# ziyangwang007/CV-SSL-MIS

Hardware: AMD Instinct MI355X
Metric: training images-or-volumes/sec/node (Mean-Teacher step) (higher is better)
Workload: dtype f32

## Files before the change

### cv-ssl-mis_amd/csrc/conv_wino.hip

```cpp
#include "common.h"
#include "wino.h"
#include <stdio.h>
#include <stdlib.h>
#include <type_traits>

namespace {

using namespace mis_dma;
using namespace mis_wino;

struct WinoArgs {
    const float* x; long long x_bs;
    const float* wt;
    const float* bias;
    float* y; long long y_bs;
    int N, Cin, Cout, D, H, W;
    int nci4;
    int boxes_z, boxes_y, boxes_x, co_groups;
    unsigned n_blocks, n_blocks_padded;
    float2* stat; long long stat_sc, stat_sn;
    const float* xn; long long xn_bs;
    const float* thr;
    float slope;
    int ks; long long y_ks;
};

template <int GZ_, int GY_, int GX_, int WZ_, int WY_, int WX_, int COB_, int NBUF_, int DW_ = 0, int FLAT_ = 0>
struct WinoCfg {
    static constexpr int GZ = GZ_, GY = GY_, GX = GX_, WZ = WZ_, WY = WY_, WX = WX_, COB = COB_, NBUF = NBUF_, FLAT = FLAT_;
    static constexpr int BZ = GZ * WZ, BY = GY * WY, BX = GX * WX;
    static constexpr int OZ = 2 * BZ, OY = 2 * BY, OX = 2 * BX;
    static constexpr int HZ = OZ + 2, HY = OY + 2;
    static constexpr int DW = DW_;
    static constexpr int NQ = DW ? OX + 2 : (OX + 8) / 4, RX = DW ? OX + 2 : NQ * 4, X0 = DW ? 0 : 3;
    static constexpr int GROUPS = HZ * HY * NQ;
    static constexpr int NCH = (GROUPS + 63) / 64;
    static constexpr int CS_RAW = DW ? NCH * 64 : GROUPS * 4;
    static constexpr int CS = CS_RAW + (49 - CS_RAW % 64 + 64) % 64;
    static constexpr int IN_FLOATS = 4 * CS;
    static constexpr int W_FLOATS = COB * 4096;
    static constexpr int STAGE = IN_FLOATS + W_FLOATS;
    static constexpr int MAX_COUT = 384;
    static constexpr int LDS_BYTES = NBUF * STAGE * 4 + 512 + MAX_COUT * 4 + NCH * 256;
    static constexpr int WPW = COB * 4;
    static constexpr int P = NCH + WPW;
    static_assert(FLAT ? (GZ * GY * GX <= 64 && WZ * WY * WX == 1 && COB == 1 && DW == 1) : (GZ * GY * GX == 16), "16 tiles per wave");
    static_assert(FLAT || WZ * WY * WX * COB == 4, "4 waves");
    static_assert(NBUF == 3 || NBUF == 4, "ring depth");
    static_assert(2 * P <= 63 && P <= 21, "vmcnt range (two stages in flight), DMA slots");
    static_assert(LDS_BYTES <= 160 * 1024, "LDS");
};

#ifndef MIS_WINO_DBG_CT
#define MIS_WINO_DBG_CT 0
#endif
#ifndef MIS_WINO_NV
#define MIS_WINO_NV 16
#endif
constexpr int NVP = MIS_WINO_NV;
constexpr int DBG = MIS_WINO_DBG_CT;

extern __shared__ __attribute__((aligned(16))) float mis_wino_lds[];

template <class C>
struct Issue {
    unsigned voff[C::NCH];
    unsigned wvoff[C::WPW];
    i32x4 rx, rw;
    unsigned st;
    unsigned cbase;
    unsigned wbase;

    template <int I>
    __device__ __forceinline__ void piece(int wave) const {
        if constexpr (I >= 0 && I < C::NCH && !(DBG & 256)) {
            if constexpr (C::DW) {
                dma_dword_s(st + (unsigned)(wave * C::CS + I * 64) * 4u, voff[I], cbase, rx);
            } else if (I * 64 + 64 <= C::GROUPS || I * 64 + (int)(threadIdx.x & 63) < C::GROUPS) {
                dma_dwordx4_s(st + (unsigned)(wave * C::CS + I * 256) * 4u, voff[I], cbase, rx);
            }
        } else if constexpr (I >= C::NCH && I < C::P && !(DBG & 128)) {
            dma_dwordx4_s(st + (unsigned)(C::IN_FLOATS + (wave + 4 * (I - C::NCH)) * 256) * 4u, wvoff[I - C::NCH], wbase, rw);
        }
    }
    template <int I, int END>
    __device__ __forceinline__ void pieces(int wave) const {
        if constexpr (I < END) { piece<I>(wave); pieces<I + 1, END>(wave); }
    }
};

typedef const __attribute__((address_space(3))) float* lds_ptr;
struct RawPlanes { lds_ptr z[4]; };

template <class C, bool FIRST, int K>
__device__ __forceinline__ void slots(const f32x4* __restrict__ wl, const f32x4* __restrict__ wl_next,
                                      const RawPlanes& raw, const f32x2 (&cur)[32], f32x2 (&nxt)[32],
                                      f32x4 (&acc)[64], f32x4 (&ar)[4], const Issue<C>& is, int wave) {
    if constexpr (K < 64) {
        constexpr int G = K / 4;
        if constexpr (K % 4 == 0 && !(DBG & 32)) ar[(G + 2) % 4] = G < 14 ? wl[(G + 2) * 64] : wl_next[(G - 14) * 64];
        {
            const float av = ar[G % 4][K % 4], bv = cur[K / 2][K % 2];
            if constexpr (K < NVP) {
                if constexpr (FIRST) asm volatile("v_mfma_f32_16x16x4_f32 %0, %1, %2, 0" : "=v"(acc[K]) : "v"(av), "v"(bv));
                else asm volatile("v_mfma_f32_16x16x4_f32 %0, %1, %2, %0" : "+v"(acc[K]) : "v"(av), "v"(bv));
            } else {
                if constexpr (FIRST) asm volatile("v_mfma_f32_16x16x4_f32 %0, %1, %2, 0" : "=a"(acc[K]) : "v"(av), "v"(bv));
                else asm volatile("v_mfma_f32_16x16x4_f32 %0, %1, %2, %0" : "+a"(acc[K]) : "v"(av), "v"(bv));
            }
        }
        if constexpr (K < 16 && !(DBG & 16)) {
#pragma unroll
            for (int j = 2 * K; j < 2 * K + 2; ++j) {
                const int z = j / 8, y = (j / 2) % 4, xp = j % 2;
                nxt[j] = f32x2{raw.z[z][y * C::RX + 2 * xp], raw.z[z][y * C::RX + 2 * xp + 1]};
            }
        }
        constexpr int SP = C::P <= 12 ? 5 : 3;
        if constexpr (K >= 2 && (K - 2) % SP == 0 && (K - 2) / SP < C::P && !(DBG & 8)) is.template piece<(K - 2) / SP>(wave);
        if constexpr (K >= 16 && K < 40 && !(DBG & 16) && (DBG & 512)) in_unit<K - 16>(nxt);
        __builtin_amdgcn_sched_barrier(0);
        slots<C, FIRST, K + 1>(wl, wl_next, raw, cur, nxt, acc, ar, is, wave);
    }
}

template <class C, bool NB, bool SPLIT>
__device__ __forceinline__ void wino_fwd_body(const WinoArgs& a) {
    float* const lds = mis_wino_lds;
    const int xcd = blockIdx.x % MIS_NUM_XCD, slot = blockIdx.x / MIS_NUM_XCD, nslot = gridDim.x / MIS_NUM_XCD;
    const unsigned per = a.n_blocks_padded / MIS_NUM_XCD;
    const unsigned box_end = (xcd + 1) * per < a.n_blocks ? (xcd + 1) * per : a.n_blocks;
    unsigned box = xcd * per + slot;
    if (box >= box_end) return;

    const int tid = threadIdx.x, lane = tid & 63;
    const int wave = __builtin_amdgcn_readfirstlane(tid >> 6);
    const int lk = lane >> 4, lj = lane & 15;
    const int cb = wave % C::COB, grp = wave / C::COB;
    int tx, ty, tz;
    bool lane_live = true;
    if constexpr (C::FLAT) {
        int t = grp * 16 + lj;
        lane_live = t < C::BZ * C::BY * C::BX;
        t = lane_live ? t : 0;
        tx = t % C::BX; ty = (t / C::BX) % C::BY; tz = t / (C::BX * C::BY);
    } else {
        const int gx = grp % C::WX, gy = (grp / C::WX) % C::WY, gz = grp / (C::WX * C::WY);
        tx = gx * C::GX + lj % C::GX; ty = gy * C::GY + (lj / C::GX) % C::GY; tz = gz * C::GZ + lj / (C::GX * C::GY);
    }
    const long long S = (long long)a.D * a.H * a.W;
    const unsigned s_bytes = (unsigned)S * 4u;
    const unsigned lds0 = lds_addr(lds);
    const int nst = SPLIT ? a.nci4 / a.ks : a.nci4;

    struct Box { int cg, kz, bx, by, bz, n, z0, y0, x0; long long idx; };
    auto finish = [&](Box& b) {
        b.z0 = b.bz * C::OZ; b.y0 = b.by * C::OY; b.x0 = b.bx * C::OX;
        b.idx = ((long long)b.bz * a.boxes_y + b.by) * a.boxes_x + b.bx;
    };
    auto decode = [&](unsigned L) {
        Box b;
        unsigned t = L;
        b.cg = t % a.co_groups; t /= a.co_groups;
        b.kz = 0;
        if constexpr (SPLIT) { b.kz = t % a.ks; t /= a.ks; }
        b.bx = t % a.boxes_x;   t /= a.boxes_x;
        b.by = t % a.boxes_y;   t /= a.boxes_y;
        b.bz = t % a.boxes_z;   t /= a.boxes_z;
        b.n = t;
        finish(b);
        return b;
    };
    const Box stride = decode((unsigned)nslot);
    auto advance = [&](Box b) {
        int c;
        b.cg += stride.cg;     c = b.cg >= a.co_groups; b.cg -= c ? a.co_groups : 0;
        if constexpr (SPLIT) { b.kz += stride.kz + c; c = b.kz >= a.ks; b.kz -= c ? a.ks : 0; }
        b.bx += stride.bx + c; c = b.bx >= a.boxes_x;   b.bx -= c ? a.boxes_x : 0;
        b.by += stride.by + c; c = b.by >= a.boxes_y;   b.by -= c ? a.boxes_y : 0;
        b.bz += stride.bz + c; c = b.bz >= a.boxes_z;   b.bz -= c ? a.boxes_z : 0;
        b.n += stride.n + c;
        finish(b);
        return b;
    };

    Issue<C> is;
    is.rw = make_rsrc(a.wt, (unsigned)a.co_groups * C::COB * (unsigned)a.nci4 * 16384u);
#pragma unroll
    for (int i = 0; i < C::WPW; ++i) {
        const int j = wave + 4 * i, b = j / 16, pp = j % 16;
        is.wvoff[i] = (unsigned)((b * a.nci4) * 4096 + pp * 256 + lane * 4) * 4u;
    }
    int icg = 0, ikz = 0;
    unsigned* const s_geo = reinterpret_cast<unsigned*>(lds + C::NBUF * C::STAGE + 128 + C::MAX_COUT);
    if (tid < 64) {
#pragma unroll
        for (int p = 0; p < C::NCH; ++p) {
            const int e = p * 64 + tid;
            const int row = e / C::NQ, q = e - row * C::NQ;
            const int hz = row / C::HY, hy = row - hz * C::HY;
            s_geo[p * 64 + tid] = (unsigned)(hz | hy << 4 | q << 9 | (e < C::GROUPS ? 1 << 14 : 0));
        }
    }
    __syncthreads();
    auto cursor_box = [&](const Box& b_in, bool live) {
        Box b = b_in;
        if (DBG & 2048) { b.n = 0; b.z0 = 0; b.y0 = 0; b.x0 = 0; }
        icg = b.cg; ikz = b.kz;
        is.rx = make_rsrc(a.x + (long long)b.n * a.x_bs, live ? (unsigned)a.Cin * s_bytes : 0u);
        unsigned geo[C::NCH];
#pragma unroll
        for (int p = 0; p < C::NCH; ++p) geo[p] = s_geo[p * 64 + lane];
        __builtin_amdgcn_sched_barrier(0);
#pragma unroll
        for (int p = 0; p < C::NCH; ++p) {
            const unsigned g = geo[p];
            const int qz = b.z0 - 1 + (int)(g & 15u), qy = b.y0 - 1 + (int)((g >> 4) & 31u);
            const int qx = C::DW ? b.x0 - 1 + (int)((g >> 9) & 31u) : b.x0 - 4 + 4 * (int)((g >> 9) & 31u);
            const bool ok = (g >> 14) && (unsigned)qz < (unsigned)a.D && (unsigned)qy < (unsigned)a.H &&
                            (unsigned)qx < (unsigned)a.W;
            is.voff[p] = ok ? (unsigned)((qz * a.H + qy) * a.W + qx) * 4u : OOB;
        }
    };
    auto cursor_set = [&](unsigned gs_issue, int istage) {
        is.st = lds0 + (gs_issue % C::NBUF) * (unsigned)(C::STAGE * 4);
        if constexpr (SPLIT) istage += ikz * nst;
        is.cbase = (unsigned)(istage * 4 + wave) * s_bytes;
        is.wbase = (unsigned)(icg * C::COB * a.nci4 + istage) * 16384u;
    };

    const int poff = ((2 * tz) * C::HY + 2 * ty) * C::RX + C::X0 + 2 * tx + lk * C::CS;
    auto raw_of = [&](unsigned gs) { return lds + (gs % C::NBUF) * C::STAGE + poff; };
    auto wl_of = [&](unsigned gs) {
        return reinterpret_cast<const f32x4*>(lds + (gs % C::NBUF) * C::STAGE + C::IN_FLOATS + cb * 4096) + lane;
    };

    float* const s_bias = lds + C::NBUF * C::STAGE + 128;
    if constexpr (NB) {
        for (int i = tid; i < a.N * a.Cout; i += 256) s_bias[i] = a.thr[i];
    } else {
        for (int i = tid; i < a.Cout; i += 256) s_bias[i] = a.bias ? a.bias[i] : 0.f;
    }
    constexpr int A = C::NBUF - 1;
    const unsigned nslot_u = (unsigned)nslot;
    Box bb = decode(box), nb = bb;
    cursor_box(bb, true);
#pragma unroll
    for (int s = 0; s < A; ++s) { cursor_set((unsigned)s, s); is.template pieces<0, C::P>(wave); }
    static_assert(A == 3, "the waits below are written for a ring of 4");
    vmwait<2 * C::P>::go();
    __syncthreads();
    f32x2 ua[32], ub[32];
    f32x4 acc[64];
    f32x4 ar[4];
    {
        const float* __restrict__ raw = raw_of(0);
#pragma unroll
        for (int j = 0; j < 32; ++j) {
            const int z = j / 8, y = (j / 2) % 4, xp = j % 2;
            ua[j] = f32x2{raw[(z * C::HY + y) * C::RX + 2 * xp], raw[(z * C::HY + y) * C::RX + 2 * xp + 1]};
        }
    }
    ar[0] = wl_of(0)[0]; ar[1] = wl_of(0)[64];
    in_units<0, 24>(ua);
    vmwait<C::P>::go();
    __syncthreads();

    unsigned gs = 0;
    const int sw = nst - A;
    auto iter = [&](auto first, f32x2 (&cur)[32], f32x2 (&nxt)[32], int s, bool relaxed) {
        cursor_set(gs + A, s + A < nst ? s + A : s + A - nst);
        RawPlanes rp;
        {
            const float* r0 = raw_of(gs + 1);
#pragma unroll
            for (int z = 0; z < 4; ++z) {
                rp.z[z] = (lds_ptr)r0 + z * C::HY * C::RX;
                asm volatile("" : "+v"(rp.z[z]));
            }
        }
        slots<C, decltype(first)::value, 0>(wl_of(gs), wl_of(gs + 1), rp, cur, nxt, acc, ar, is, wave);
        if (!(DBG & 16) && !(DBG & 512)) in_units<0, 24>(nxt);
        ++gs;
        if (NB && relaxed) vmwait<C::P + 16>::go();
        else vmwait<(DBG & 1024) ? 2 * C::P : C::P>::go();
        if (!(DBG & 64)) __syncthreads();
    };

    float run1[4] = {0.f, 0.f, 0.f, 0.f}, run2[4] = {0.f, 0.f, 0.f, 0.f};
    f32x2 xv[NB ? 16 : 1];
    for (; box < box_end; box += nslot_u, bb = nb) {
        const bool nlive = box + nslot_u < box_end;
        nb = advance(bb);
        if (sw == 0 && !(DBG & 4)) cursor_box(nb, nlive);
        iter(std::true_type{}, ua, ub, 0, false);
        if (sw == 1 && !(DBG & 4)) cursor_box(nb, nlive);
        iter(std::false_type{}, ub, ua, 1, false);
        for (int s = 2; s < nst; s += 2) {
            if (sw == s && !(DBG & 4)) cursor_box(nb, nlive);
            if constexpr (NB) {
                if (s + 2 >= nst && !(DBG & 4096)) {
                    const int oz = bb.z0 + 2 * tz, oy = bb.y0 + 2 * ty, ox = bb.x0 + 2 * tx;
                    const bool okx = lane_live && oz < a.D && oy < a.H && ox < a.W;
                    const int c0 = (bb.cg * C::COB + cb) * 16;
                    const i32x4 rxn = make_rsrc(a.xn + (long long)bb.n * a.xn_bs + (long long)c0 * S, 16u * s_bytes);
                    const unsigned vx = okx ? (unsigned)(lk * 4) * s_bytes + (unsigned)((oz * a.H + oy) * a.W + ox) * 4u : OOB;
                    unsigned vzy[4];
#pragma unroll
                    for (int zy = 0; zy < 4; ++zy) vzy[zy] = vx + (unsigned)(((zy >> 1) * a.H + (zy & 1)) * a.W) * 4u;
#pragma unroll
                    for (int r = 0; r < 4; ++r) {
                        const unsigned so = (unsigned)r * s_bytes;
#pragma unroll
                        for (int zy = 0; zy < 4; ++zy)
                            asm volatile("buffer_load_dwordx2 %0, %1, %2, %3 offen"
                                         : "=v"(xv[r * 4 + zy]) : "v"(vzy[zy]), "s"(rxn), "s"(so) : "memory");
                    }
                }
            }
            iter(std::false_type{}, ua, ub, s, NB && s + 2 >= nst);
            if (sw == s + 1 && !(DBG & 4)) cursor_box(nb, nlive);
            iter(std::false_type{}, ub, ua, s + 1, false);
        }

        if constexpr (NB) {
#pragma unroll
            for (int i = 0; i < 16; ++i) asm volatile("" : "+v"(xv[i]));
        }
        if (DBG & 2) continue;
        asm volatile("s_nop 15\n\ts_nop 15" ::: "memory");
        const int oz = bb.z0 + 2 * tz, oy = bb.y0 + 2 * ty, ox = bb.x0 + 2 * tx;
        const bool ok = lane_live && oz < a.D && oy < a.H && ox < a.W;
        const int co0 = (bb.cg * C::COB + cb) * 16;
        const __amdgpu_buffer_rsrc_t ry = __builtin_amdgcn_make_buffer_rsrc(
            (void*)(a.y + (SPLIT ? (long long)bb.kz * a.y_ks : 0LL) + (long long)bb.n * a.y_bs + (long long)co0 * S), 0,
            (int)(16u * s_bytes), 0x00020000);
        const unsigned vo = ok && !(DBG & 1) ? (unsigned)(lk * 4) * s_bytes + (unsigned)((oz * a.H + oy) * a.W + ox) * 4u : OOB;
#pragma unroll
        for (int h = 0; h < 2; ++h) {
            f32x2 o[2][2][2];
#pragma unroll
            for (int x = 0; x < 4; ++x) {
                f32x2 py[2][2];
#pragma unroll
                for (int y = 0; y < 4; ++y) {
                    const f32x2 m0 = (y * 4 + x < NVP) ? f32x2{acc[y * 4 + x][2 * h], acc[y * 4 + x][2 * h + 1]} : acc_pair(acc[y * 4 + x], h),
                                m1 = acc_pair(acc[16 + y * 4 + x], h),
                                m2 = acc_pair(acc[32 + y * 4 + x], h), m3 = acc_pair(acc[48 + y * 4 + x], h);
                    const f32x2 pz0 = m0 + m1 + m2, pz1 = m1 - m2 - m3;
                    if (y == 0) { py[0][0] = pz0; py[1][0] = pz1; }
                    if (y == 1) { py[0][0] += pz0; py[1][0] += pz1; py[0][1] = pz0; py[1][1] = pz1; }
                    if (y == 2) { py[0][0] += pz0; py[1][0] += pz1; py[0][1] -= pz0; py[1][1] -= pz1; }
                    if (y == 3) { py[0][1] -= pz0; py[1][1] -= pz1; }
                    __builtin_amdgcn_sched_barrier(0);
                }
#pragma unroll
                for (int zz = 0; zz < 2; ++zz)
#pragma unroll
                    for (int yy = 0; yy < 2; ++yy) {
                        if (x == 0) { o[zz][yy][0] = py[zz][yy]; }
                        if (x == 1) { o[zz][yy][0] += py[zz][yy]; o[zz][yy][1] = py[zz][yy]; }
                        if (x == 2) { o[zz][yy][0] += py[zz][yy]; o[zz][yy][1] -= py[zz][yy]; }
                        if (x == 3) { o[zz][yy][1] -= py[zz][yy]; }
                    }
                __builtin_amdgcn_sched_barrier(0);
            }
            f32x2 bv = *reinterpret_cast<const f32x2*>(s_bias + (NB ? bb.n * a.Cout : 0) + co0 + lk * 4 + 2 * h);
            const f32x2 th = bv;
            if constexpr (NB) bv = f32x2{0.f, 0.f};
            f32x2 s1 = {0.f, 0.f}, s2 = s1;
#pragma unroll
            for (int zz = 0; zz < 2; ++zz)
#pragma unroll
                for (int yy = 0; yy < 2; ++yy) {
                    const f32x2 v0 = o[zz][yy][0] + bv, v1 = o[zz][yy][1] + bv;
                    if constexpr (NB && !(DBG & 8192)) {
#pragma unroll
                        for (int rr = 0; rr < 2; ++rr) {
                            const f32x2 x = xv[(2 * h + rr) * 4 + zz * 2 + yy];
                            const float d0 = x[0] > th[rr] ? v0[rr] : v0[rr] * a.slope;
                            const float d1 = x[1] > th[rr] ? v1[rr] : v1[rr] * a.slope;
                            s1[rr] += d0 + d1;
                            s2[rr] = fmaf(d0, x[0], fmaf(d1, x[1], s2[rr]));
                        }
                    } else {
                        s1 += v0 + v1;
                        s2 += v0 * v0 + v1 * v1;
                    }
#pragma unroll
                    for (int rr = 0; rr < 2; ++rr) {
                        typedef unsigned u32x2 __attribute__((ext_vector_type(2)));
                        const f32x2 v = {v0[rr], v1[rr]};
                        __builtin_amdgcn_raw_buffer_store_b64(__builtin_bit_cast(u32x2, v), ry,
                                                              (int)(vo + (unsigned)((zz * a.H + yy) * a.W) * 4u),
                                                              (int)((unsigned)(2 * h + rr) * s_bytes), 0);
                    }
                }
            if constexpr (C::DW) {
                if (!ok) { s1 = f32x2{0.f, 0.f}; s2 = s1; }
            }
            run1[2 * h] += s1[0]; run1[2 * h + 1] += s1[1]; run2[2 * h] += s2[0]; run2[2 * h + 1] += s2[1];
            __builtin_amdgcn_sched_barrier(0);
        }
        const bool flush = !nlive || nb.n != bb.n || nb.cg != bb.cg;
        if (a.stat && !flush) {
            if (tid < C::COB * 16)
                a.stat[(long long)(bb.cg * C::COB * 16 + tid) * a.stat_sc + (long long)bb.n * a.stat_sn + bb.idx] = make_float2(0.f, 0.f);
        } else if (a.stat) {
            float st1[4], st2[4];
#pragma unroll
            for (int r = 0; r < 4; ++r) { st1[r] = run1[r]; st2[r] = run2[r]; run1[r] = 0.f; run2[r] = 0.f; }
#pragma unroll
            for (int r = 0; r < 4; ++r)
#pragma unroll
                for (int o = 1; o < 16; o <<= 1) {
                    st1[r] += __shfl_xor(st1[r], o, 64);
                    st2[r] += __shfl_xor(st2[r], o, 64);
                }
            float2* red = reinterpret_cast<float2*>(lds + C::NBUF * C::STAGE);
            if (lj == 0) {
#pragma unroll
                for (int r = 0; r < 4; ++r) red[wave * 16 + lk * 4 + r] = make_float2(st1[r], st2[r]);
            }
            __syncthreads();
            if (tid < C::COB * 16) {
                const int b = tid / 16, c = tid % 16;
                float sx = 0.f, sq = 0.f;
#pragma unroll
                for (int g = 0; g < 4 / C::COB; ++g) {
                    const float2 p = red[(g * C::COB + b) * 16 + c];
                    sx += p.x; sq += p.y;
                }
                a.stat[(long long)((bb.cg * C::COB + b) * 16 + c) * a.stat_sc + (long long)bb.n * a.stat_sn + bb.idx] =
                    make_float2(sx, sq);
            }
        }
    }
}

template <class C, bool NB = false>
__global__ __launch_bounds__(256) __attribute__((amdgpu_waves_per_eu(1, 1))) void wino_fwd_kernel(const WinoArgs a) {
    wino_fwd_body<C, NB, false>(a);
}
template <class C>
__global__ __launch_bounds__(256) __attribute__((amdgpu_waves_per_eu(1, 1))) void wino_fwd_split_kernel(const WinoArgs a) {
    wino_fwd_body<C, false, true>(a);
}

template <class C, bool NB = false, bool SPLIT = false>
int launch_wino(WinoArgs a, hipStream_t stream) {
    a.boxes_z = (int)mis_cdiv(a.D, C::OZ);
    a.boxes_y = (int)mis_cdiv(a.H, C::OY);
    a.boxes_x = (int)mis_cdiv(a.W, C::OX);
    a.co_groups = a.Cout / (16 * C::COB);
    const long long nb = (long long)a.N * a.boxes_z * a.boxes_y * a.boxes_x * a.co_groups * (SPLIT ? a.ks : 1);
    if (nb <= 0 || nb > 0x7fffffffLL) return MIS_ERR_ARG;
    a.n_blocks = (unsigned)nb;
    a.n_blocks_padded = (unsigned)(mis_cdiv(nb, MIS_NUM_XCD) * MIS_NUM_XCD);
    static std::atomic<unsigned long long> attr_done{0};
    const unsigned grid = a.n_blocks_padded < 256u ? a.n_blocks_padded : 256u;
    if constexpr (SPLIT) {
        if (mis_set_lds_attr(reinterpret_cast<const void*>(&wino_fwd_split_kernel<C>), C::LDS_BYTES, attr_done) != MIS_OK)
            return MIS_ERR_LAUNCH;
        hipLaunchKernelGGL((wino_fwd_split_kernel<C>), dim3(grid), dim3(256), C::LDS_BYTES, stream, a);
    } else {
        if (mis_set_lds_attr(reinterpret_cast<const void*>(&wino_fwd_kernel<C, NB>), C::LDS_BYTES, attr_done) != MIS_OK)
            return MIS_ERR_LAUNCH;
        hipLaunchKernelGGL((wino_fwd_kernel<C, NB>), dim3(grid), dim3(256), C::LDS_BYTES, stream, a);
    }
    return mis_launch_status();
}

using WinoV2 = WinoCfg<1, 4, 4, 4, 1, 1, 1, 4, 1>;
using WinoV3 = WinoCfg<3, 3, 6, 1, 1, 1, 1, 4, 1, 1>;

int wino_splits(int N, int Cin, int Cout, int D, int H, int W, int variant) {
    static const bool on = [] { const char* e = getenv("MIS_WINO_SPLIT"); return !(e && e[0] == '0'); }();
    if (!on || (variant != 2 && variant != 3)) return 1;
    const long long boxes = variant == 2 ? mis_cdiv(D, 8) * mis_cdiv(H, 8) * mis_cdiv(W, 8) : (long long)(D / 6) * (H / 6) * (W / 12);
    const long long entries = (long long)N * boxes * (Cout / 16);
    const int nst = (Cin + 3) / 4;
    int ks = 1;
    while (entries * ks < 192 && ks < 8 && nst % (2 * ks) == 0 && nst / (2 * ks) >= 8 && (nst / (2 * ks)) % 2 == 0) ks *= 2;
    return ks;
}

__global__ __launch_bounds__(256) void wino_split_reduce_kernel(const float* __restrict__ part, long long part_ks, long long part_bs,
                                                                const float* __restrict__ bias, float* __restrict__ y,
                                                                long long y_bs, int Cout, int S, int ks, float2* stat,
                                                                long long stat_sc, long long stat_sn, int tiles) {
    __shared__ float2 red[256];
    const int n = blockIdx.x / Cout, c = blockIdx.x - n * Cout;
    const float* __restrict__ p = part + (long long)n * part_bs + (long long)c * S;
    float* __restrict__ o = y + (long long)n * y_bs + (long long)c * S;
    const float b = bias ? bias[c] : 0.f;
    float s1 = 0.f, s2 = 0.f;
    for (int v = threadIdx.x; v < S; v += 256) {
        float acc = p[v];
        for (int k = 1; k < ks; ++k) acc += p[(long long)k * part_ks + v];
        acc += b;
        o[v] = acc;
        s1 += acc; s2 = fmaf(acc, acc, s2);
    }
    if (!stat) return;
    red[threadIdx.x] = make_float2(s1, s2);
    __syncthreads();
    for (int w = 128; w > 0; w >>= 1) {
        if ((int)threadIdx.x < w) { red[threadIdx.x].x += red[threadIdx.x + w].x; red[threadIdx.x].y += red[threadIdx.x + w].y; }
        __syncthreads();
    }
    for (int t = threadIdx.x; t < tiles; t += 256)
        stat[(long long)c * stat_sc + (long long)n * stat_sn + t] = t == 0 ? red[0] : make_float2(0.f, 0.f);
}

}

extern "C" int mis_conv3d_wino_select(int N, int Cin, int Cout, int D, int H, int W) {
    if (N <= 0 || Cin < 16 || Cin % 8 || Cout <= 0 || Cout % 16 || Cout > 384 || D <= 0 || H <= 0 || W <= 0) return -1;
    if (D % 2 || H % 2 || W % 2) return -1;
    if (((long long)Cin + 32) * D * H * W * 4 >= (1LL << 30)) return -1;
    if (W % 32 == 0 && D % 4 == 0 && H % 4 == 0) return 0;
    if (W % 16 == 0 && D % 4 == 0 && H % 8 == 0) return 1;
    if (W % 8 == 0 && D % 8 == 0 && H % 8 == 0 && Cin >= 32) return 2;
    if (W == 12 && D % 6 == 0 && H % 6 == 0 && Cin >= 32 &&
        (long long)N * (D / 6) * (H / 6) * (Cout / 16) * wino_splits(N, Cin, Cout, D, H, W, 3) >= 64) return 3;
    if (Cin >= 32) {
        const long long boxes = mis_cdiv(D, 8) * mis_cdiv(H, 8) * mis_cdiv(W, 8);
        if ((long long)D * H * W * 5 >= boxes * 512 * 2 && (long long)N * boxes * (Cout / 16) * wino_splits(N, Cin, Cout, D, H, W, 2) >= 128)
            return 2;
    }
    return -1;
}

namespace {
template <class C>
long long boxes_per_image(int D, int H, int W) {
    return mis_cdiv(D, C::OZ) * mis_cdiv(H, C::OY) * mis_cdiv(W, C::OX);
}
}

extern "C" long long mis_conv3d_wino_stat_tiles(int D, int H, int W, int variant) {
    if (D <= 0 || H <= 0 || W <= 0) return MIS_ERR_ARG;
    if (variant == 0) return boxes_per_image<WinoCfg<1, 1, 16, 2, 2, 1, 1, 4>>(D, H, W);
    if (variant == 1) return boxes_per_image<WinoCfg<1, 2, 8, 2, 2, 1, 1, 4>>(D, H, W);
    if (variant == 2) return boxes_per_image<WinoCfg<1, 4, 4, 4, 1, 1, 1, 4, 1>>(D, H, W);
    if (variant == 3) return boxes_per_image<WinoCfg<3, 3, 6, 1, 1, 1, 1, 4, 1, 1>>(D, H, W);
    return MIS_ERR_UNSUPPORTED;
}

extern "C" int mis_conv3d_wino_kernel_name(int variant, char* name, int name_len) {
    if (!name || name_len <= 0) return MIS_ERR_ARG;
    if (variant == 0) snprintf(name, name_len, "wino_fwd_kernel<WinoCfg<1, 1, 16, 2, 2, 1, 1, 4, 0, 0>, false>");
    else if (variant == 1) snprintf(name, name_len, "wino_fwd_kernel<WinoCfg<1, 2, 8, 2, 2, 1, 1, 4, 0, 0>, false>");
    else if (variant == 2) snprintf(name, name_len, "wino_fwd_kernel<WinoCfg<1, 4, 4, 4, 1, 1, 1, 4, 1, 0>, false>");
    else if (variant == 3) snprintf(name, name_len, "wino_fwd_kernel<WinoCfg<3, 3, 6, 1, 1, 1, 1, 4, 1, 1>, false>");
    else return MIS_ERR_UNSUPPORTED;
    return MIS_OK;
}

extern "C" int mis_conv3d_wino_fwd(const float* x, long long x_bs, const float* wt, const float* bias, float* y,
                                   long long y_bs, int N, int Cin, int Cout, int D, int H, int W, float* stat,
                                   long long stat_sc, long long stat_sn, int variant, hipStream_t stream) {
    if (!x || !wt || !y || N <= 0 || Cin <= 0 || Cout <= 0 || D <= 0 || H <= 0 || W <= 0) return MIS_ERR_ARG;
    const long long S = (long long)D * H * W;
    if (x_bs < (long long)Cin * S || y_bs < (long long)Cout * S) return MIS_ERR_ARG;
    if (Cout % 16 || Cout > 384 || Cin % 8 || Cin < 16 || (W % 4 && variant < 2) || D % 2 || H % 2 || W % 2 || y_bs % 2 || ((uintptr_t)y & 7) || ((uintptr_t)wt & 15))
        return MIS_ERR_UNSUPPORTED;
    if (((long long)Cin + 32) * S * 4 >= (1LL << 30)) return MIS_ERR_UNSUPPORTED;
    WinoArgs a{};
    a.x = x; a.x_bs = x_bs; a.wt = wt; a.bias = bias; a.y = y; a.y_bs = y_bs;
    a.N = N; a.Cin = Cin; a.Cout = Cout; a.D = D; a.H = H; a.W = W;
    a.nci4 = (Cin + 3) / 4;
    a.stat = reinterpret_cast<float2*>(stat); a.stat_sc = stat_sc; a.stat_sn = stat_sn;
    if (variant == 0) return launch_wino<WinoCfg<1, 1, 16, 2, 2, 1, 1, 4>>(a, stream);
    if (variant == 1) return launch_wino<WinoCfg<1, 2, 8, 2, 2, 1, 1, 4>>(a, stream);
    if (variant == 2) return launch_wino<WinoCfg<1, 4, 4, 4, 1, 1, 1, 4, 1>>(a, stream);
    if (variant == 3) {
        if (W != 12 || D % 6 || H % 6) return MIS_ERR_UNSUPPORTED;
        return launch_wino<WinoCfg<3, 3, 6, 1, 1, 1, 1, 4, 1, 1>>(a, stream);
    }
    return MIS_ERR_UNSUPPORTED;
}

extern "C" int mis_conv3d_wino_fwd_splits(int N, int Cin, int Cout, int D, int H, int W, int variant) {
    if (N <= 0 || Cin <= 0 || Cout <= 0 || D <= 0 || H <= 0 || W <= 0 || variant < 0 || variant > 3) return MIS_ERR_ARG;
    return wino_splits(N, Cin, Cout, D, H, W, variant);
}
extern "C" long long mis_conv3d_wino_fwd_workspace_bytes(int N, int Cin, int Cout, int D, int H, int W, int variant) {
    const int ks = mis_conv3d_wino_fwd_splits(N, Cin, Cout, D, H, W, variant);
    if (ks < 0) return ks;
    return ks > 1 ? (long long)ks * N * Cout * D * H * W * 4 : 0;
}

extern "C" int mis_conv3d_wino_fwd_ws(const float* x, long long x_bs, const float* wt, const float* bias, float* y,
                                      long long y_bs, int N, int Cin, int Cout, int D, int H, int W, float* stat,
                                      long long stat_sc, long long stat_sn, int variant, float* workspace,
                                      long long workspace_bytes, hipStream_t stream) {
    const int ks = mis_conv3d_wino_fwd_splits(N, Cin, Cout, D, H, W, variant);
    if (ks < 0) return ks;
    if (ks == 1)
        return mis_conv3d_wino_fwd(x, x_bs, wt, bias, y, y_bs, N, Cin, Cout, D, H, W, stat, stat_sc, stat_sn, variant, stream);
    if (!x || !wt || !y || !workspace) return MIS_ERR_ARG;
    const long long S = (long long)D * H * W;
    if (x_bs < (long long)Cin * S || y_bs < (long long)Cout * S) return MIS_ERR_ARG;
    if (Cout % 16 || Cout > 384 || Cin % 8 || Cin < 16 || D % 2 || H % 2 || W % 2 || ((uintptr_t)workspace & 15) || ((uintptr_t)wt & 15))
        return MIS_ERR_UNSUPPORTED;
    if (variant == 3 && (W != 12 || D % 6 || H % 6)) return MIS_ERR_UNSUPPORTED;
    if (((long long)Cin + 32) * S * 4 >= (1LL << 30)) return MIS_ERR_UNSUPPORTED;
    if (workspace_bytes < (long long)ks * N * Cout * S * 4) return MIS_ERR_WORKSPACE;
    WinoArgs a{};
    a.x = x; a.x_bs = x_bs; a.wt = wt; a.bias = nullptr; a.y = workspace; a.y_bs = (long long)Cout * S;
    a.N = N; a.Cin = Cin; a.Cout = Cout; a.D = D; a.H = H; a.W = W;
    a.nci4 = (Cin + 3) / 4;
    a.ks = ks; a.y_ks = (long long)N * Cout * S;
    const int st = variant == 2 ? launch_wino<WinoV2, false, true>(a, stream) : launch_wino<WinoV3, false, true>(a, stream);
    if (st) return st;
    const int tiles = (int)mis_conv3d_wino_stat_tiles(D, H, W, variant);
    hipLaunchKernelGGL(wino_split_reduce_kernel, dim3((unsigned)(N * Cout)), dim3(256), 0, stream, workspace, a.y_ks, a.y_bs, bias, y,
                       y_bs, Cout, (int)S, ks, reinterpret_cast<float2*>(stat), stat_sc, stat_sn, tiles);
    return mis_launch_status();
}

extern "C" int mis_conv3d_wino_dgrad_norm(const float* dy, long long dy_bs, const float* wt, float* da, long long da_bs,
                                          int N, int Cin, int Cout, int D, int H, int W, const float* xn, long long xn_bs,
                                          const float* mean, float slope, float* part, long long part_sc,
                                          long long part_sn, int variant, hipStream_t stream) {
    if (!dy || !wt || !da || !xn || !mean || !part || N <= 0 || Cin <= 0 || Cout <= 0 || D <= 0 || H <= 0 || W <= 0)
        return MIS_ERR_ARG;
    const long long S = (long long)D * H * W;
    if (dy_bs < (long long)Cin * S || da_bs < (long long)Cout * S || xn_bs < (long long)Cout * S) return MIS_ERR_ARG;
    if (variant < 0 || variant > 1 || (long long)N * Cout > 384) return MIS_ERR_UNSUPPORTED;
    if (Cout % 16 || Cin % 8 || Cin < 16 || W % 4 || D % 2 || H % 2 || da_bs % 2 || xn_bs % 2 || ((uintptr_t)da & 7) ||
        ((uintptr_t)xn & 7) || ((uintptr_t)wt & 15))
        return MIS_ERR_UNSUPPORTED;
    if (mis_conv3d_wino_select(N, Cin, Cout, D, H, W) != variant) return MIS_ERR_UNSUPPORTED;
    if (((long long)Cin + 32) * S * 4 >= (1LL << 30) || 16 * S * 4 >= (1LL << 31)) return MIS_ERR_UNSUPPORTED;
    WinoArgs a{};
    a.x = dy; a.x_bs = dy_bs; a.wt = wt; a.bias = nullptr; a.y = da; a.y_bs = da_bs;
    a.N = N; a.Cin = Cin; a.Cout = Cout; a.D = D; a.H = H; a.W = W;
    a.nci4 = (Cin + 3) / 4;
    a.stat = reinterpret_cast<float2*>(part); a.stat_sc = part_sc; a.stat_sn = part_sn;
    a.xn = xn; a.xn_bs = xn_bs; a.thr = mean; a.slope = slope;
    if (variant == 0) return launch_wino<WinoCfg<1, 1, 16, 2, 2, 1, 1, 4>, true>(a, stream);
    return launch_wino<WinoCfg<1, 2, 8, 2, 2, 1, 1, 4>, true>(a, stream);
}
```

### include/mis_hip.h

```cpp
#ifndef MIS_HIP_H
#define MIS_HIP_H

#include <stdint.h>

#ifdef __cplusplus
extern "C" {
#endif

#define MIS_OK 0
#define MIS_ERR_ARG (-1)
#define MIS_ERR_UNSUPPORTED (-2)
#define MIS_ERR_LAUNCH (-3)
#define MIS_ERR_WORKSPACE (-4)

#ifdef MIS_HIP_BUILD
typedef hipStream_t mis_stream_t;
#else
typedef void* mis_stream_t;
#endif

typedef struct MisStepState {
    uint64_t seed;
    uint64_t offset;
    int64_t iter_num;
    float lr;
    float ema_alpha;
    float cons_weight;
    float cons_gate;
} MisStepState;

int mis_abi_version(void);

int mis_conv_cin_pad(int cin);
int mis_conv_cout_pad(int cout);
long long mis_conv_packed_floats(int Cout, int Cin, int taps, int mode);
int mis_conv_pack_weights(const float* w, float* wp, int Cout, int Cin, int taps, int mode, mis_stream_t stream);
int mis_conv_pack_job_bytes(void);
long long mis_conv_pack_job(void* job_out, const float* w, float* wp, int Cout, int Cin, int taps, int mode,
                            long long start);
int mis_conv_pack_batch(const void* jobs_device, int n, long long total_floats, mis_stream_t stream);
int mis_conv_fwd(const float* x, long long x_bs, const float* wp, const float* bias, float* y, long long y_bs,
                 int N, int Cin, int Cout, int D, int H, int W, int kd, int kh, int kw, mis_stream_t stream);
long long mis_conv_fwd_stat_tiles(int N, int Cin, int Cout, int D, int H, int W, int kd, int kh, int kw);
int mis_conv_fwd_stats(const float* x, long long x_bs, const float* wp, const float* bias, float* y, long long y_bs,
                       int N, int Cin, int Cout, int D, int H, int W, int kd, int kh, int kw, float* stat,
                       long long stat_sc, long long stat_sn, mis_stream_t stream);
int mis_norm_stats_finalize(const float* part, int N, int C, long long S, int tiles, int per_sample, float eps,
                            float* mean, float* rstd, float* running_mean, float* running_var,
                            long long* num_batches_tracked, float momentum, mis_stream_t stream);
int mis_conv_fwd_kernel_name(int N, int Cin, int Cout, int D, int H, int W, int kd, int kh, int kw, char* name,
                             int name_len);
int mis_conv3d_wino_select(int N, int Cin, int Cout, int D, int H, int W);
long long mis_conv3d_wino_stat_tiles(int D, int H, int W, int variant);
int mis_conv3d_wino_kernel_name(int variant, char* name, int name_len);
int mis_conv3d_wino_fwd(const float* x, long long x_bs, const float* wt, const float* bias, float* y, long long y_bs,
                        int N, int Cin, int Cout, int D, int H, int W, float* stat, long long stat_sc,
                        long long stat_sn, int variant, mis_stream_t stream);
int mis_conv3d_wino_fwd_splits(int N, int Cin, int Cout, int D, int H, int W, int variant);
long long mis_conv3d_wino_fwd_workspace_bytes(int N, int Cin, int Cout, int D, int H, int W, int variant);
int mis_conv3d_wino_fwd_ws(const float* x, long long x_bs, const float* wt, const float* bias, float* y, long long y_bs,
                           int N, int Cin, int Cout, int D, int H, int W, float* stat, long long stat_sc, long long stat_sn,
                           int variant, float* workspace, long long workspace_bytes, mis_stream_t stream);
int mis_conv3d_wino_dgrad_norm(const float* dy, long long dy_bs, const float* wt, float* da, long long da_bs, int N,
                               int Cin, int Cout, int D, int H, int W, const float* xn, long long xn_bs,
                               const float* mean, float slope, float* part, long long part_sc, long long part_sn,
                               int variant, mis_stream_t stream);
int mis_conv2d_wino_select(int N, int Cin, int Cout, int H, int W);
long long mis_conv2d_wino_stat_tiles(int H, int W, int variant);
int mis_conv2d_wino_kernel_name(int variant, char* name, int name_len);
int mis_conv2d_wino_fwd(const float* x, long long x_bs, const float* wt, const float* bias, float* y, long long y_bs,
                        int N, int Cin, int Cout, int H, int W, float* stat, long long stat_sc, long long stat_sn,
                        int variant, mis_stream_t stream);
int mis_conv2d_wino_wgrad_select(int N, int Cin, int Cout, int H, int W);
int mis_conv2d_wino_wgrad_kernel_name(int variant, char* name, int name_len);
long long mis_conv2d_wino_wgrad_workspace_bytes(int N, int Cin, int Cout, int H, int W, int variant);
int mis_conv2d_wino_wgrad(const float* x, long long x_bs, const float* dy, long long dy_bs, float* dw, float* workspace,
                          long long workspace_bytes, int N, int Cin, int Cout, int H, int W, int accumulate, int variant,
                          mis_stream_t stream);
int mis_conv3d_wino_wgrad_select(int N, int Cin, int Cout, int D, int H, int W);
int mis_conv3d_wino_wgrad_kernel_name(int variant, char* name, int name_len);
long long mis_conv3d_wino_wgrad_workspace_bytes(int N, int Cin, int Cout, int D, int H, int W, int variant);
int mis_conv3d_wino_wgrad(const float* x, long long x_bs, const float* dy, long long dy_bs, float* dw, float* workspace,
                          long long workspace_bytes, int N, int Cin, int Cout, int D, int H, int W, int accumulate,
                          int variant, mis_stream_t stream);
long long mis_conv_wgrad_workspace_bytes(int N, int Cin, int Cout, int D, int H, int W, int kd, int kh, int kw);
int mis_conv_wgrad_kernel_name(int N, int Cin, int Cout, int D, int H, int W, int kd, int kh, int kw, char* name,
                               int name_len);
int mis_conv_wgrad(const float* x, long long x_bs, const float* dy, long long dy_bs, float* dw, float* workspace,
                   long long workspace_bytes, int N, int Cin, int Cout, int D, int H, int W, int kd, int kh,
                   int kw, int accumulate, mis_stream_t stream);
int mis_channel_sum(const float* x, long long x_bs, int N, int C, long long S, float* out, int accumulate,
                    void* workspace, long long workspace_bytes, mis_stream_t stream);

long long mis_norm_workspace_bytes(int N, int C, long long S, int per_sample);
int mis_norm_stats(const float* x, long long x_bs, int N, int C, long long S, int per_sample, float eps,
                   float* mean, float* rstd, float* running_mean, float* running_var,
                   long long* num_batches_tracked, float momentum, void* workspace, long long workspace_bytes,
                   mis_stream_t stream);
int mis_norm_stats_from_running(const float* running_mean, const float* running_var, float eps, float* mean,
                                float* rstd, int C, mis_stream_t stream);
int mis_norm_act_fwd(const float* x, long long x_bs, float* y, long long y_bs, int N, int C, long long S,
                     int per_sample, const float* mean, const float* rstd, const float* gamma, const float* beta,
                     float slope, float drop_p, unsigned drop_salt, const MisStepState* state,
                     const float* drop_mask, mis_stream_t stream);
int mis_norm_act_bwd(const float* x, long long x_bs, const float* da, long long da_bs, float* dx, long long dx_bs,
                     int N, int C, long long S, int per_sample, const float* mean, const float* rstd,
                     const float* gamma, const float* beta, float slope, float drop_p, unsigned drop_salt,
                     const MisStepState* state, const float* drop_mask, float* dgamma, float* dbeta,
                     int accumulate_affine, void* workspace, long long workspace_bytes, mis_stream_t stream);
int mis_norm_act_fwd_g(const float* x, long long x_bs, float* y, long long y_bs, int N, int C, long long S,
                       int per_sample, int cg, const float* mean, const float* rstd, const float* gamma,
                       const float* beta, float slope, float drop_p, unsigned drop_salt, const MisStepState* state,
                       const float* drop_mask, mis_stream_t stream);
int mis_norm_act_bwd_g(const float* x, long long x_bs, const float* da, long long da_bs, float* dx, long long dx_bs,
                       int N, int C, long long S, int per_sample, int cg, int no_norm, const float* mean,
                       const float* rstd, const float* gamma, const float* beta, float slope, float drop_p,
                       unsigned drop_salt, const MisStepState* state, const float* drop_mask, float* dgamma,
                       float* dbeta, int accumulate_affine, void* workspace, long long workspace_bytes,
                       mis_stream_t stream);

int mis_norm_act_bwd_sums(const float* x, long long x_bs, const float* da, long long da_bs, int N, int C, long long S,
                          int per_sample, const float* mean, const float* rstd, const float* gamma, const float* beta,
                          float slope, float* sums, float* dgamma, float* dbeta, int accumulate_affine, void* workspace,
                          long long workspace_bytes, mis_stream_t stream);
int mis_norm_act_bwd_tiles(const float* x, long long x_bs, const float* da, long long da_bs, float* dx, long long dx_bs,
                           int N, int C, long long S, const float* mean, const float* rstd, float slope,
                           const float* part, int tiles, float* sums, mis_stream_t stream);
int mis_norm_res_act_fwd(const float* x, long long x_bs, const float* res, long long res_bs, float* y, long long y_bs,
                         int N, int C, long long S, int per_sample, const float* mean, const float* rstd,
                         const float* gamma, const float* beta, float slope, int add_after_act, mis_stream_t stream);
int mis_norm_res_act_bwd(const float* x, long long x_bs, const float* res, long long res_bs, const float* dy,
                         long long dy_bs, float* dx, long long dx_bs, float* dres, long long dres_bs, int accumulate_dres,
                         int N, int C, long long S, int per_sample, const float* mean, const float* rstd,
                         const float* gamma, const float* beta, float slope, float* dgamma, float* dbeta,
                         int accumulate_affine, int add_after_act, void* workspace, long long workspace_bytes,
                         mis_stream_t stream);
int mis_conv_wgrad_cin1_norm_eligible(int N, int Cout, int D, int H, int W);
int mis_conv_wgrad_cin1_norm(const float* x, long long x_bs, const float* da, long long da_bs, const float* y,
                             long long y_bs, int N, int D, int H, int W, int per_sample, const float* mean,
                             const float* rstd, const float* gamma, const float* beta, const float* sums, float slope,
                             float* dw, float* workspace, long long workspace_bytes, int accumulate,
                             mis_stream_t stream);

int mis_norm_head_eligible(int C, int K);
long long mis_norm_head_workspace_bytes(int N, int C, long long S, int per_sample, int K);
int mis_norm_head_fwd(const float* x, long long x_bs, int N, int C, long long S, int per_sample, const float* mean,
                      const float* rstd, const float* gamma, const float* beta, float slope, float drop_p,
                      unsigned drop_salt, const MisStepState* state, const float* drop_mask, const float* w,
                      const float* b, int K, float* logits, long long l_bs, unsigned long long* drop_bits,
                      mis_stream_t stream);
int mis_norm_head_bwd(const float* x, long long x_bs, const float* dlogits, long long dl_bs, float* dx, long long dx_bs,
                      int N, int C, long long S, int per_sample, const float* mean, const float* rstd,
                      const float* gamma, const float* beta, float slope, float drop_p, unsigned drop_salt,
                      const MisStepState* state, const float* drop_mask, const float* w, int K, float* dgamma,
                      float* dbeta, int accumulate_affine, float* dw, float* db, int accumulate_w,
                      const unsigned long long* drop_bits, void* workspace, long long workspace_bytes,
                      mis_stream_t stream);

int mis_norm_act_fwd_pool(const float* x, long long x_bs, float* y, long long y_bs, float* pooled, long long p_bs,
                          unsigned char* idx, int N, int C, int D, int H, int W, int per_sample, int cg,
                          const float* mean, const float* rstd, const float* gamma, const float* beta, float slope,
                          float drop_p, unsigned drop_salt, const MisStepState* state, const float* drop_mask,
                          mis_stream_t stream);
int mis_norm_act_bwd_pool(const float* x, long long x_bs, const float* da, long long da_bs, const float* dpool,
                          long long dp_bs, const unsigned char* idx, float* dx, long long dx_bs, int N, int C, int D,
                          int H, int W, int per_sample, int cg, const float* mean, const float* rstd,
                          const float* gamma, const float* beta, float slope, float drop_p, unsigned drop_salt,
                          const MisStepState* state, const float* drop_mask, float* dgamma, float* dbeta,
                          int accumulate_affine, void* workspace, long long workspace_bytes, mis_stream_t stream);

int mis_maxpool2_fwd(const float* x, long long x_bs, float* y, long long y_bs, unsigned char* idx, int N, int C,
                     int D, int H, int W, mis_stream_t stream);
int mis_maxpool2_bwd(const float* dy, long long dy_bs, const unsigned char* idx, float* dx, long long dx_bs,
                     int N, int C, int D, int H, int W, int accumulate, mis_stream_t stream);
int mis_upsample2_fwd(const float* x, long long x_bs, float* y, long long y_bs, int N, int C, int D, int H,
                      int W, int align_corners, mis_stream_t stream);
int mis_upsample2_bwd(const float* dy, long long dy_bs, float* dx, long long dx_bs, int N, int C, int D, int H,
                      int W, int align_corners, int accumulate, mis_stream_t stream);

long long mis_loss_tail_workspace_bytes(int B, int C, long long S);
int mis_loss_tail(const float* student, long long s_bs, const float* teacher, long long t_bs, const void* label,
                  int label_bytes, int B, int L, int C, long long S, float cons_weight,
                  const MisStepState* state, float loss_scale, float* out, float* dlogits, long long d_bs,
                  void* workspace, long long workspace_bytes, mis_stream_t stream);

long long mis_cross_teaching_tail_workspace_bytes(int B, int C, long long S);
int mis_cross_pseudo_tail(const float* own, long long s_bs, const float* other, long long o_bs, const void* label,
                          int label_bytes, int B, int L, int C, long long S, float cons_weight,
                          const MisStepState* state, int pseudo_ce, float* out, float* dlogits, long long d_bs,
                          void* workspace, long long workspace_bytes, mis_stream_t stream);
int mis_cross_pseudo_mt_tail(const float* own, long long s_bs, const float* other, long long o_bs,
                             const float* teacher, long long t_bs, const void* label, int label_bytes, int B, int L,
                             int C, long long S, float cons_weight, float mt_weight, const MisStepState* state,
                             int pseudo_ce, float* out, float* dlogits, long long d_bs, void* workspace,
                             long long workspace_bytes, mis_stream_t stream);
int mis_cross_teaching_tail(const float* own, long long s_bs, const float* other, long long o_bs, const void* label,
                            int label_bytes, int B, int L, int C, long long S, float cons_weight,
                            const MisStepState* state, float* out, float* dlogits, long long d_bs, void* workspace,
                            long long workspace_bytes, mis_stream_t stream);

int mis_softmax_mean_accumulate(const float* logits, long long l_bs, float* acc, long long a_bs, int U, int R, int C,
                                long long S, float scale, int first, mis_stream_t stream);
long long mis_uamt_tail_workspace_bytes(int B, int C, long long S);
int mis_uamt_tail(const float* student, long long s_bs, const float* teacher, long long t_bs, const float* mean_probs,
                  long long mp_bs, const void* label, int label_bytes, int B, int L, int C, long long S,
                  float cons_weight, const MisStepState* state, long long iter_num, double max_iterations,
// ... 276 lines not shown
```

Before: 470.6.

## Keep Winograd filter resident in LDS when channel count fits the ring

Adds a ResidentFilter config for variant 0. When the input-channel chunks exactly fill the ring (Cin/4 == NBUF) and Cout is 16, the filter slices are loaded once per buffer at kernel start, and the per-stage DMA issue covers only the input pieces (PS = NCH). This removes repeated weight DMA traffic and shortens the vmcnt waits in the pipelined loop. It also derives the dword halo-row layout from an LDS budget check and renames the template flag to NARROW, at the cost of extra template instantiations and a kernel-name encoding change.

```diff
diff --git a/cv-ssl-mis_amd/csrc/conv_wino.hip b/cv-ssl-mis_amd/csrc/conv_wino.hip
--- a/cv-ssl-mis_amd/csrc/conv_wino.hip
+++ b/cv-ssl-mis_amd/csrc/conv_wino.hip
@@ -25,30 +25,42 @@
     int ks; long long y_ks;
 };
 
-template <int GZ_, int GY_, int GX_, int WZ_, int WY_, int WX_, int COB_, int NBUF_, int DW_ = 0, int FLAT_ = 0>
+constexpr int wino_pad49(int raw) { return raw + (49 - raw % 64 + 64) % 64; }
+constexpr int WINO_MAX_COUT = 384, WINO_LDS_LIMIT = 160 * 1024;
+constexpr int wino_lds_bytes(int nbuf, int cs, int cob, int nch) { return nbuf * (4 * cs + cob * 4096) * 4 + 512 + WINO_MAX_COUT * 4 + nch * 256; }
+
+template <int GZ_, int GY_, int GX_, int WZ_, int WY_, int WX_, int COB_, int NBUF_, int NARROW_ = 0, int FLAT_ = 0>
 struct WinoCfg {
     static constexpr int GZ = GZ_, GY = GY_, GX = GX_, WZ = WZ_, WY = WY_, WX = WX_, COB = COB_, NBUF = NBUF_, FLAT = FLAT_;
     static constexpr int BZ = GZ * WZ, BY = GY * WY, BX = GX * WX;
     static constexpr int OZ = 2 * BZ, OY = 2 * BY, OX = 2 * BX;
     static constexpr int HZ = OZ + 2, HY = OY + 2;
-    static constexpr int DW = DW_;
+    static constexpr int NARROW = NARROW_;
+    static constexpr int GROUPS16 = HZ * HY * ((OX + 8) / 4);
+    static constexpr int DW = NARROW && wino_lds_bytes(NBUF, wino_pad49(GROUPS16 * 4), COB, (GROUPS16 + 63) / 64) > WINO_LDS_LIMIT;
     static constexpr int NQ = DW ? OX + 2 : (OX + 8) / 4, RX = DW ? OX + 2 : NQ * 4, X0 = DW ? 0 : 3;
     static constexpr int GROUPS = HZ * HY * NQ;
     static constexpr int NCH = (GROUPS + 63) / 64;
     static constexpr int CS_RAW = DW ? NCH * 64 : GROUPS * 4;
-    static constexpr int CS = CS_RAW + (49 - CS_RAW % 64 + 64) % 64;
+    static constexpr int CS = wino_pad49(CS_RAW);
     static constexpr int IN_FLOATS = 4 * CS;
     static constexpr int W_FLOATS = COB * 4096;
     static constexpr int STAGE = IN_FLOATS + W_FLOATS;
-    static constexpr int MAX_COUT = 384;
-    static constexpr int LDS_BYTES = NBUF * STAGE * 4 + 512 + MAX_COUT * 4 + NCH * 256;
+    static constexpr int MAX_COUT = WINO_MAX_COUT;
+    static constexpr int LDS_BYTES = wino_lds_bytes(NBUF, CS, COB, NCH);
     static constexpr int WPW = COB * 4;
     static constexpr int P = NCH + WPW;
-    static_assert(FLAT ? (GZ * GY * GX <= 64 && WZ * WY * WX == 1 && COB == 1 && DW == 1) : (GZ * GY * GX == 16), "16 tiles per wave");
+    static constexpr int RF = 0, PS = P;
+    static_assert(FLAT ? (GZ * GY * GX <= 64 && WZ * WY * WX == 1 && COB == 1 && NARROW == 1) : (GZ * GY * GX == 16), "16 tiles per wave");
     static_assert(FLAT || WZ * WY * WX * COB == 4, "4 waves");
     static_assert(NBUF == 3 || NBUF == 4, "ring depth");
     static_assert(2 * P <= 63 && P <= 21, "vmcnt range (two stages in flight), DMA slots");
-    static_assert(LDS_BYTES <= 160 * 1024, "LDS");
+    static_assert(LDS_BYTES <= WINO_LDS_LIMIT, "LDS");
+};
+
+template <class C>
+struct ResidentFilter : C {
+    static constexpr int RF = 1, PS = C::NCH;
 };
 
 #ifndef MIS_WINO_DBG_CT
@@ -117,7 +129,7 @@
             }
         }
         constexpr int SP = C::P <= 12 ? 5 : 3;
-        if constexpr (K >= 2 && (K - 2) % SP == 0 && (K - 2) / SP < C::P && !(DBG & 8)) is.template piece<(K - 2) / SP>(wave);
+        if constexpr (K >= 2 && (K - 2) % SP == 0 && (K - 2) / SP < C::PS && !(DBG & 8)) is.template piece<(K - 2) / SP>(wave);
         if constexpr (K >= 16 && K < 40 && !(DBG & 16) && (DBG & 512)) in_unit<K - 16>(nxt);
         __builtin_amdgcn_sched_barrier(0);
         slots<C, FIRST, K + 1>(wl, wl_next, raw, cur, nxt, acc, ar, is, wave);
@@ -245,10 +257,14 @@
     const unsigned nslot_u = (unsigned)nslot;
     Box bb = decode(box), nb = bb;
     cursor_box(bb, true);
-#pragma unroll
-    for (int s = 0; s < A; ++s) { cursor_set((unsigned)s, s); is.template pieces<0, C::P>(wave); }
+    if constexpr (C::RF) {
+#pragma unroll
+        for (int c = 0; c < C::NBUF; ++c) { cursor_set((unsigned)c, c); is.template pieces<C::NCH, C::P>(wave); }
+    }
+#pragma unroll
+    for (int s = 0; s < A; ++s) { cursor_set((unsigned)s, s); is.template pieces<0, C::PS>(wave); }
     static_assert(A == 3, "the waits below are written for a ring of 4");
-    vmwait<2 * C::P>::go();
+    vmwait<2 * C::PS>::go();
     __syncthreads();
     f32x2 ua[32], ub[32];
     f32x4 acc[64];
@@ -263,7 +279,7 @@
     }
     ar[0] = wl_of(0)[0]; ar[1] = wl_of(0)[64];
     in_units<0, 24>(ua);
-    vmwait<C::P>::go();
+    vmwait<C::PS>::go();
     __syncthreads();
 
     unsigned gs = 0;
@@ -282,8 +298,8 @@
         slots<C, decltype(first)::value, 0>(wl_of(gs), wl_of(gs + 1), rp, cur, nxt, acc, ar, is, wave);
         if (!(DBG & 16) && !(DBG & 512)) in_units<0, 24>(nxt);
         ++gs;
-        if (NB && relaxed) vmwait<C::P + 16>::go();
-        else vmwait<(DBG & 1024) ? 2 * C::P : C::P>::go();
+        if (NB && relaxed) vmwait<C::PS + 16>::go();
+        else vmwait<(DBG & 1024) ? 2 * C::PS : C::PS>::go();
         if (!(DBG & 64)) __syncthreads();
     };
 
@@ -396,7 +412,7 @@
                                                               (int)((unsigned)(2 * h + rr) * s_bytes), 0);
                     }
                 }
-            if constexpr (C::DW) {
+            if constexpr (C::NARROW) {
                 if (!ok) { s1 = f32x2{0.f, 0.f}; s2 = s1; }
             }
             run1[2 * h] += s1[0]; run1[2 * h + 1] += s1[1]; run2[2 * h] += s2[0]; run2[2 * h + 1] += s2[1];
@@ -471,8 +487,15 @@
     return mis_launch_status();
 }
 
+using WinoV0 = WinoCfg<1, 1, 16, 2, 2, 1, 1, 4>;
+using WinoV1 = WinoCfg<1, 2, 8, 2, 2, 1, 1, 4>;
 using WinoV2 = WinoCfg<1, 4, 4, 4, 1, 1, 1, 4, 1>;
 using WinoV3 = WinoCfg<3, 3, 6, 1, 1, 1, 1, 4, 1, 1>;
+static_assert(!WinoV0::DW && !WinoV1::DW && WinoV2::DW && !WinoV3::DW, "halo rows: single dwords at 8 x 8 x 8 only");
+
+bool wino_filter_resident(int Cin, int Cout, int variant) {
+    return variant == 0 && (Cin + 3) / 4 == WinoV0::NBUF && Cout == 16 * WinoV0::COB;
+}
 
 int wino_splits(int N, int Cin, int Cout, int D, int H, int W, int variant) {
     static const bool on = [] { const char* e = getenv("MIS_WINO_SPLIT"); return !(e && e[0] == '0'); }();
@@ -541,15 +564,21 @@
 
 extern "C" long long mis_conv3d_wino_stat_tiles(int D, int H, int W, int variant) {
     if (D <= 0 || H <= 0 || W <= 0) return MIS_ERR_ARG;
-    if (variant == 0) return boxes_per_image<WinoCfg<1, 1, 16, 2, 2, 1, 1, 4>>(D, H, W);
-    if (variant == 1) return boxes_per_image<WinoCfg<1, 2, 8, 2, 2, 1, 1, 4>>(D, H, W);
-    if (variant == 2) return boxes_per_image<WinoCfg<1, 4, 4, 4, 1, 1, 1, 4, 1>>(D, H, W);
-    if (variant == 3) return boxes_per_image<WinoCfg<3, 3, 6, 1, 1, 1, 1, 4, 1, 1>>(D, H, W);
+    if (variant == 0) return boxes_per_image<WinoV0>(D, H, W);
+    if (variant == 1) return boxes_per_image<WinoV1>(D, H, W);
+    if (variant == 2) return boxes_per_image<WinoV2>(D, H, W);
+    if (variant == 3) return boxes_per_image<WinoV3>(D, H, W);
     return MIS_ERR_UNSUPPORTED;
 }
 
 extern "C" int mis_conv3d_wino_kernel_name(int variant, char* name, int name_len) {
-    if (!name || name_len <= 0) return MIS_ERR_ARG;
+    if (!name || name_len <= 0 || variant < 0) return MIS_ERR_ARG;
+    const int Cin = (variant >> 4) & 0xfff, Cout = variant >> 16;
+    variant &= 15;
+    if (wino_filter_resident(Cin, Cout, variant)) {
+        snprintf(name, name_len, "wino_fwd_kernel<ResidentFilter<WinoCfg<1, 1, 16, 2, 2, 1, 1, 4, 0, 0> >, false>");
+        return MIS_OK;
+    }
     if (variant == 0) snprintf(name, name_len, "wino_fwd_kernel<WinoCfg<1, 1, 16, 2, 2, 1, 1, 4, 0, 0>, false>");
     else if (variant == 1) snprintf(name, name_len, "wino_fwd_kernel<WinoCfg<1, 2, 8, 2, 2, 1, 1, 4, 0, 0>, false>");
     else if (variant == 2) snprintf(name, name_len, "wino_fwd_kernel<WinoCfg<1, 4, 4, 4, 1, 1, 1, 4, 1, 0>, false>");
@@ -572,12 +601,13 @@
     a.N = N; a.Cin = Cin; a.Cout = Cout; a.D = D; a.H = H; a.W = W;
     a.nci4 = (Cin + 3) / 4;
     a.stat = reinterpret_cast<float2*>(stat); a.stat_sc = stat_sc; a.stat_sn = stat_sn;
-    if (variant == 0) return launch_wino<WinoCfg<1, 1, 16, 2, 2, 1, 1, 4>>(a, stream);
-    if (variant == 1) return launch_wino<WinoCfg<1, 2, 8, 2, 2, 1, 1, 4>>(a, stream);
-    if (variant == 2) return launch_wino<WinoCfg<1, 4, 4, 4, 1, 1, 1, 4, 1>>(a, stream);
+    if (variant == 0 && wino_filter_resident(Cin, Cout, 0)) return launch_wino<ResidentFilter<WinoV0>>(a, stream);
+    if (variant == 0) return launch_wino<WinoV0>(a, stream);
+    if (variant == 1) return launch_wino<WinoV1>(a, stream);
+    if (variant == 2) return launch_wino<WinoV2>(a, stream);
     if (variant == 3) {
         if (W != 12 || D % 6 || H % 6) return MIS_ERR_UNSUPPORTED;
-        return launch_wino<WinoCfg<3, 3, 6, 1, 1, 1, 1, 4, 1, 1>>(a, stream);
+        return launch_wino<WinoV3>(a, stream);
     }
     return MIS_ERR_UNSUPPORTED;
 }
@@ -641,6 +671,7 @@
     a.nci4 = (Cin + 3) / 4;
     a.stat = reinterpret_cast<float2*>(part); a.stat_sc = part_sc; a.stat_sn = part_sn;
     a.xn = xn; a.xn_bs = xn_bs; a.thr = mean; a.slope = slope;
-    if (variant == 0) return launch_wino<WinoCfg<1, 1, 16, 2, 2, 1, 1, 4>, true>(a, stream);
-    return launch_wino<WinoCfg<1, 2, 8, 2, 2, 1, 1, 4>, true>(a, stream);
-}
+    if (variant == 0 && wino_filter_resident(Cin, Cout, 0)) return launch_wino<ResidentFilter<WinoV0>, true>(a, stream);
+    if (variant == 0) return launch_wino<WinoV0, true>(a, stream);
+    return launch_wino<WinoV1, true>(a, stream);
+}
diff --git a/include/mis_hip.h b/include/mis_hip.h
--- a/include/mis_hip.h
+++ b/include/mis_hip.h
@@ -52,6 +52,7 @@
                              int name_len);
 int mis_conv3d_wino_select(int N, int Cin, int Cout, int D, int H, int W);
 long long mis_conv3d_wino_stat_tiles(int D, int H, int W, int variant);
+#define MIS_WINO_LAUNCH(variant, Cin, Cout) ((variant) | (Cin) << 4 | (Cout) << 16)
 int mis_conv3d_wino_kernel_name(int variant, char* name, int name_len);
 int mis_conv3d_wino_fwd(const float* x, long long x_bs, const float* wt, const float* bias, float* y, long long y_bs,
                         int N, int Cin, int Cout, int D, int H, int W, float* stat, long long stat_sc,
```

New measurement: 481.4 (median of 6 runs). 1.02x the previous value.
